# zhaoyuhsin/Edge-Guided-Near-Eye-Image-Analysis-for-Head-Mounted-Displays

Measured on AMD Instinct MI355X. Metric: eye-frames/sec (320x240): inference edge+seg (value), +fit, exact fp32, and train fwd+bwd at 1 MI355X, higher is better.
Workload: dtype f32 tensors; inference products split into f16 hi/lo pairs (3 f16 MFMAs per product, 22-bit significand), f32 accumulate (`exact_fp32`: every product on the f32 MFMA); `train`: bf16 storage, f32 accumulate, f32 master weights (and an f32-storage leg)

## Files before the change

edge-guided-near-eye-image-analysis-for-head-mounted-displays_amd/csrc/conv1x1_f16.hip:

```cpp
#include "common.h"
#include "kernel_util.h"
#include "split_f16.h"

namespace {

__device__ __forceinline__ void split8(const u32x4 a, const u32x4 b, float s, h8& hi, h8& lo) {
  const f32x4 va = __builtin_bit_cast(f32x4, a), vb = __builtin_bit_cast(f32x4, b);
  const float x[8] = {va[0], va[1], va[2], va[3], vb[0], vb[1], vb[2], vb[3]};
#pragma unroll
  for (int q = 0; q < 4; ++q) {
    h2 h, l;
    egne::split2(x[2 * q], x[2 * q + 1], s, h, l);
    hi[2 * q] = h[0]; hi[2 * q + 1] = h[1];
    lo[2 * q] = l[0]; lo[2 * q + 1] = l[1];
  }
}

template <int TN, bool UP = false>
__global__ __launch_bounds__(256) void conv1x1_f16x3_kernel(const egne_conv_desc p, const _Float16* __restrict__ fhi,
                                                            const _Float16* __restrict__ flo, float a_scale, float out_scale,
                                                            int G, long long M, int nblocks) {
  extern __shared__ __attribute__((aligned(16))) _Float16 wl[];
  const int tid = threadIdx.x, lane = tid & 63, wave = tid >> 6;
  const int li = lane & 31, kq = lane >> 5;
  const int NT = p.CoutP >> 5, nt0 = blockIdx.y * TN;
  for (int it = tid; it < G * TN * 2 * 64; it += 256) {
    const int l = it & 63, hl = (it >> 6) & 1;
    const int tn = (it >> 7) % TN, g = (it >> 7) / TN;
    const _Float16* src = (hl ? flo : fhi) + (((long long)g * NT + nt0 + tn) * 64 + l) * 8;
    *(u32x4*)&wl[(long long)it * 8] = *(const u32x4*)src;
  }
  __syncthreads();
  constexpr int UPC = 18, UPP = 32 * TN + 8;
  [[maybe_unused]] float* const patch = (float*)(wl + (long long)G * TN * 2 * 64 * 8) + wave * (UPC * UPP);

  const float slope = p.act == EGNE_ACT_RELU ? 0.f : (p.act == EGNE_ACT_LEAKY ? 0.01f : 1.f);
  f32x4 bias[TN][4];
#pragma unroll
  for (int tn = 0; tn < TN; ++tn)
#pragma unroll
    for (int j = 0; j < 4; ++j) {
      const int n = (nt0 + tn) * 32 + 8 * j + 4 * kq;
      bias[tn][j] = (p.bias && n < p.Cout_store) ? *(const f32x4*)(p.bias + n) : (f32x4)(0.f);
    }

  for (int blk = blockIdx.x * 4 + wave; blk < nblocks; blk += gridDim.x * 4) {
    const long long m0 = (long long)blk * 32;
    const long long rows = M - m0 < 32 ? M - m0 : 32;
    f32x16 acc[TN];
#pragma unroll
    for (int tn = 0; tn < TN; ++tn) acc[tn] = (f32x16)(0.f);
    int g = 0;
    for (int s = 0; s < p.nseg; ++s) {
      const egne_seg sg = p.seg[s];
      const __amdgpu_buffer_rsrc_t r = make_rsrc(sg.ptr + m0 * sg.pix_stride, (unsigned)(rows * sg.pix_stride * 4));
      const int voff = (li * (int)sg.pix_stride + sg.ch_off + 4 * kq) * 4;
      const int n16 = (sg.Cp + 15) >> 4;
      const bool tail8 = (sg.Cp & 15) != 0;
      for (int g0 = 0; g0 < n16; g0 += 4) {
        u32x4 xa[4], xb[4];
#pragma unroll
        for (int u = 0; u < 4; ++u) {
          const int gg = g0 + u;
          const int oa = gg < n16 ? voff : (int)OOB;
          const int ob = (gg < n16 && !(tail8 && gg == n16 - 1)) ? voff : (int)OOB;
          xa[u] = __builtin_amdgcn_raw_buffer_load_b128(r, oa, gg * 64, 0);
          xb[u] = __builtin_amdgcn_raw_buffer_load_b128(r, ob + 32, gg * 64, 0);
        }
#pragma unroll
        for (int u = 0; u < 4; ++u) {
          if (g0 + u < n16) {
            h8 ah, al;
            split8(xa[u], xb[u], a_scale, ah, al);
            const _Float16* wp = wl + ((long long)(g + g0 + u) * TN * 2 * 64 + lane) * 8;
#pragma unroll
            for (int tn = 0; tn < TN; ++tn) {
              const h8 wh = *(const h8*)(wp + (tn * 2 + 0) * 512), wo = *(const h8*)(wp + (tn * 2 + 1) * 512);
              acc[tn] = __builtin_amdgcn_mfma_f32_32x32x16_f16(wh, al, acc[tn], 0, 0, 0);
              acc[tn] = __builtin_amdgcn_mfma_f32_32x32x16_f16(wo, ah, acc[tn], 0, 0, 0);
              acc[tn] = __builtin_amdgcn_mfma_f32_32x32x16_f16(wh, ah, acc[tn], 0, 0, 0);
            }
          }
        }
      }
      g += n16;
    }
    const __amdgpu_buffer_rsrc_t ro = make_rsrc(p.out + m0 * p.out_pix_stride, (unsigned)(rows * p.out_pix_stride * 4));
    bool bad = false;
    [[maybe_unused]] int o00 = 0, o01 = 0, o10 = 0, o11 = 0;
    [[maybe_unused]] float w00 = 0.f, w01 = 0.f, w10 = 0.f, w11 = 0.f;
    [[maybe_unused]] __amdgpu_buffer_rsrc_t rres = ro;
    [[maybe_unused]] bool pix_ok = false, staged = false;
    if constexpr (UP) {
      const int ph = p.Ho, pw = p.Wo, hw = p.H * p.W;
      const long long m = m0 + li;
      pix_ok = m < M;
      const int b = pix_ok ? (int)(m / hw) : 0;
      const int r = pix_ok ? (int)(m - (long long)b * hw) : 0;
      const int y = r / p.W, x = r - y * p.W;
      float sy = 0.5f * (y + 0.5f) - 0.5f, sx = 0.5f * (x + 0.5f) - 0.5f;
      sy = sy < 0.f ? 0.f : sy; sx = sx < 0.f ? 0.f : sx;
      const int y0 = (int)sy, x0 = (int)sx, y1 = y0 + (y0 < ph - 1 ? 1 : 0), x1 = x0 + (x0 < pw - 1 ? 1 : 0);
      const float ly = sy - y0, lx = sx - x0;
      w00 = (1.f - ly) * (1.f - lx); w01 = (1.f - ly) * lx; w10 = ly * (1.f - lx); w11 = ly * lx;
      const int rs = (int)p.res_pix_stride, base = b * ph * pw;
      rres = make_rsrc(p.residual, (unsigned)((long long)p.B * ph * pw * rs * 4));
      const int r0 = (int)(m0 % hw), xb0 = r0 % p.W;
      staged = rows == 32 && xb0 + 32 <= p.W;
      if (staged) {
        const int bb = (int)(m0 / hw), yb = r0 / p.W;
        float syb = 0.5f * (yb + 0.5f) - 0.5f; syb = syb < 0.f ? 0.f : syb;
        const int yb0 = (int)syb, yb1 = yb0 + (yb0 < ph - 1 ? 1 : 0);
        const float lyb = syb - yb0;
        float sxb = 0.5f * (xb0 + 0.5f) - 0.5f; sxb = sxb < 0.f ? 0.f : sxb;
        const int cb = (int)sxb;
        constexpr int VPP = 8 * TN;
        for (int it = lane; it < UPC * VPP; it += 64) {
          const int cc = it / VPP, c4 = it - cc * VPP;
          const int gx = cb + cc < pw ? cb + cc : pw - 1;
          const int n = nt0 * 32 + c4 * 4;
          const int o0 = n < p.Cout_store ? (((bb * ph + yb0) * pw + gx) * rs + p.res_ch_off + n) * 4 : (int)OOB;
          const int o1 = n < p.Cout_store ? (((bb * ph + yb1) * pw + gx) * rs + p.res_ch_off + n) * 4 : (int)OOB;
          const f32x4 ra = __builtin_bit_cast(f32x4, __builtin_amdgcn_raw_buffer_load_b128(rres, o0, 0, 0));
          const f32x4 rb = __builtin_bit_cast(f32x4, __builtin_amdgcn_raw_buffer_load_b128(rres, o1, 0, 0));
          *(f32x4*)&patch[cc * UPP + c4 * 4] = (1.f - lyb) * ra + lyb * rb;
        }
        asm volatile("s_waitcnt vmcnt(0) lgkmcnt(0)" ::: "memory");
        o00 = ((x0 - cb) * UPP) * 4; o01 = ((x1 - cb) * UPP) * 4;
        w00 = 1.f - lx; w01 = lx;
      } else {
        o00 = ((base + y0 * pw + x0) * rs + p.res_ch_off) * 4; o01 = ((base + y0 * pw + x1) * rs + p.res_ch_off) * 4;
        o10 = ((base + y1 * pw + x0) * rs + p.res_ch_off) * 4; o11 = ((base + y1 * pw + x1) * rs + p.res_ch_off) * 4;
      }
    }
#pragma unroll
    for (int tn = 0; tn < TN; ++tn)
#pragma unroll
      for (int j = 0; j < 4; ++j) {
        const int n = (nt0 + tn) * 32 + 8 * j + 4 * kq;
        f32x4 v;
#pragma unroll
        for (int e = 0; e < 4; ++e) {
          const float t = acc[tn][4 * j + e] * out_scale + bias[tn][j][e];
          v[e] = fmaxf(t, t * slope);
        }
        if (tn == 0 && j == 0) bad |= egne_nonfinite(v[0]);
        if constexpr (UP) {
          if (staged) {
            const char* pb = (const char*)patch + (tn * 32 + 8 * j + 4 * kq) * 4;
            v += w00 * *(const f32x4*)(pb + o00) + w01 * *(const f32x4*)(pb + o01);
          } else {
          const bool on = pix_ok && n < p.Cout_store;
          const f32x4 a = __builtin_bit_cast(f32x4, __builtin_amdgcn_raw_buffer_load_b128(rres, on ? o00 + n * 4 : (int)OOB, 0, 0));
          const f32x4 b_ = __builtin_bit_cast(f32x4, __builtin_amdgcn_raw_buffer_load_b128(rres, on ? o01 + n * 4 : (int)OOB, 0, 0));
          const f32x4 c = __builtin_bit_cast(f32x4, __builtin_amdgcn_raw_buffer_load_b128(rres, on ? o10 + n * 4 : (int)OOB, 0, 0));
          const f32x4 d_ = __builtin_bit_cast(f32x4, __builtin_amdgcn_raw_buffer_load_b128(rres, on ? o11 + n * 4 : (int)OOB, 0, 0));
          v += w00 * a + w01 * b_ + w10 * c + w11 * d_;
          }
        }
        const int off = n < p.Cout_store ? (li * (int)p.out_pix_stride + p.out_ch_off + n) * 4 : (int)OOB;
        __builtin_amdgcn_raw_buffer_store_b128(__builtin_bit_cast(u32x4, v), ro, off, 0, 0);
      }
    egne_ovf_commit(bad, p.ovf_flag);
  }
}


template <int TN, bool STATS = false>
__global__ __launch_bounds__(256) void conv1x1_pool_f16x3_kernel(const egne_conv_desc p, const _Float16* __restrict__ fhi,
                                                                 const _Float16* __restrict__ flo, float a_scale, float out_scale,
                                                                 int G, long long M, int nblocks) {
  extern __shared__ __attribute__((aligned(16))) _Float16 wl[];
  const int tid = threadIdx.x, lane = tid & 63, wave = tid >> 6;
  const int li = lane & 31, kq = lane >> 5;
  const int NT = p.CoutP >> 5, nt0 = blockIdx.y * TN;
  for (int it = tid; it < G * TN * 2 * 64; it += 256) {
    const int l = it & 63, hl = (it >> 6) & 1;
    const int tn = (it >> 7) % TN, g = (it >> 7) / TN;
    const _Float16* src = (hl ? flo : fhi) + (((long long)g * NT + nt0 + tn) * 64 + l) * 8;
    *(u32x4*)&wl[(long long)it * 8] = *(const u32x4*)src;
  }
  __syncthreads();

  const float slope = p.act == EGNE_ACT_RELU ? 0.f : (p.act == EGNE_ACT_LEAKY ? 0.01f : 1.f);
  [[maybe_unused]] f32x4 bias[STATS ? 1 : TN][4];
  if constexpr (!STATS) {
#pragma unroll
  for (int tn = 0; tn < TN; ++tn)
#pragma unroll
    for (int j = 0; j < 4; ++j) {
      const int n = (nt0 + tn) * 32 + 8 * j + 4 * kq;
      bias[tn][j] = (p.bias && n < p.Cout_store) ? *(const f32x4*)(p.bias + n) : (f32x4)(0.f);
    }
  }
  const int H = p.H, W = p.W, Hp = p.Ho, Wp = p.Wo, hwp = Hp * Wp;
  const float s4 = 0.25f * a_scale;

  constexpr bool stats = STATS;
  const int bpf = (hwp + 31) >> 5, cb = stats ? (bpf + p.stats_nchunk - 1) / p.stats_nchunk : 1;
  constexpr int PP = 36;
  [[maybe_unused]] float* const patch = (float*)(wl + (long long)G * TN * 2 * 64 * 8) + wave * (32 * PP);
  [[maybe_unused]] const int rd = (lane >> 5) * PP + (lane & 31);

  for (int unit = blockIdx.x * 4 + wave; unit < nblocks; unit += gridDim.x * 4) {
   long long mfirst = (long long)unit * 32, mend = M;
   if (stats) {
     const int fb = unit / p.stats_nchunk, ck = unit - fb * p.stats_nchunk;
     mfirst = (long long)fb * hwp + (long long)ck * cb * 32;
     mend = (long long)(fb + 1) * hwp;
   }
   if (mend > mfirst + (long long)cb * 32) mend = mfirst + (long long)cb * 32;
   [[maybe_unused]] double ssum[TN], qsum[TN];
#pragma unroll
   for (int tn = 0; tn < TN; ++tn) ssum[tn] = qsum[tn] = 0.;
   for (long long m0 = mfirst; m0 < mend; m0 += 32) {
    const long long rows = mend - m0 < 32 ? mend - m0 : 32;
    const int b0 = (int)(m0 / hwp);
    const long long m = m0 + li;
    const bool valid = li < rows;
    const int b = valid ? (int)(m / hwp) : b0;
    const int r = (int)(m - (long long)b * hwp);
    const int yp = valid ? r / Wp : 0, xp = valid ? r - yp * Wp : 0;
    const int pin = ((b - b0) * H + 2 * yp) * W + 2 * xp;
    f32x16 acc[TN];
#pragma unroll
    for (int tn = 0; tn < TN; ++tn) acc[tn] = (f32x16)(0.f);
    int g = 0;
    for (int s = 0; s < p.nseg; ++s) {
      const egne_seg sg = p.seg[s];
      const long long frame = (long long)H * W * sg.pix_stride;
      const long long left = ((long long)p.B - b0) * frame * 4;
      const __amdgpu_buffer_rsrc_t rs = make_rsrc(sg.ptr + (long long)b0 * frame, (unsigned)(left < 2 * frame * 4 ? left : 2 * frame * 4));
      const int ps4 = (int)sg.pix_stride * 4;
      const int voff = valid ? (pin * (int)sg.pix_stride + sg.ch_off + 4 * kq) * 4 : (int)OOB;
      const float slope_in = sg.act_in == EGNE_ACT_RELU ? 0.f : (sg.act_in == EGNE_ACT_LEAKY ? 0.01f : 1.f);
      const float* tsc = sg.scale + (long long)b * sg.Cp + 4 * kq;
      const float* tsh = sg.shift + (long long)b * sg.Cp + 4 * kq;
      const int n16 = (sg.Cp + 15) >> 4;
      const bool tail8 = (sg.Cp & 15) != 0;
      for (int gg = 0; gg < n16; ++gg) {
        const bool has_b = !(tail8 && gg == n16 - 1);
        const int ob = has_b ? voff + 32 : (int)OOB;
        u32x4 xa[4], xb[4];
#pragma unroll
        for (int t = 0; t < 4; ++t) {
          const int d = ((t >> 1) * W + (t & 1)) * ps4;
          xa[t] = __builtin_amdgcn_raw_buffer_load_b128(rs, voff == (int)OOB ? (int)OOB : voff + d, gg * 64, 0);
          xb[t] = __builtin_amdgcn_raw_buffer_load_b128(rs, ob == (int)OOB ? (int)OOB : ob + d, gg * 64, 0);
        }
        const f32x4 sca = *(const f32x4*)(tsc + gg * 16), sha = *(const f32x4*)(tsh + gg * 16);
        const f32x4 scb = has_b ? *(const f32x4*)(tsc + gg * 16 + 8) : (f32x4)(0.f), shb = has_b ? *(const f32x4*)(tsh + gg * 16 + 8) : (f32x4)(0.f);
        f32x4 sa = (f32x4)(0.f), sb = (f32x4)(0.f);
#pragma unroll
        for (int t = 0; t < 4; ++t) {
          f32x4 va = __builtin_bit_cast(f32x4, xa[t]) * sca + sha, vb = __builtin_bit_cast(f32x4, xb[t]) * scb + shb;
#pragma unroll
          for (int e = 0; e < 4; ++e) { sa[e] += fmaxf(va[e], va[e] * slope_in); sb[e] += fmaxf(vb[e], vb[e] * slope_in); }
        }
        if (!valid) { sa = (f32x4)(0.f); sb = (f32x4)(0.f); }
        h8 ah, al;
        split8(__builtin_bit_cast(u32x4, sa), __builtin_bit_cast(u32x4, sb), s4, ah, al);
        const _Float16* wp = wl + ((long long)(g + gg) * TN * 2 * 64 + lane) * 8;
#pragma unroll
        for (int tn = 0; tn < TN; ++tn) {
          const h8 wh = *(const h8*)(wp + (tn * 2 + 0) * 512), wo = *(const h8*)(wp + (tn * 2 + 1) * 512);
          acc[tn] = __builtin_amdgcn_mfma_f32_32x32x16_f16(wh, al, acc[tn], 0, 0, 0);
          acc[tn] = __builtin_amdgcn_mfma_f32_32x32x16_f16(wo, ah, acc[tn], 0, 0, 0);
          acc[tn] = __builtin_amdgcn_mfma_f32_32x32x16_f16(wh, ah, acc[tn], 0, 0, 0);
        }
      }
      g += n16;
    }
    const __amdgpu_buffer_rsrc_t ro = make_rsrc(p.out + m0 * p.out_pix_stride, (unsigned)(rows * p.out_pix_stride * 4));
    bool bad = false;
#pragma unroll
    for (int tn = 0; tn < TN; ++tn)
#pragma unroll
      for (int j = 0; j < 4; ++j) {
        const int n = (nt0 + tn) * 32 + 8 * j + 4 * kq;
        f32x4 v, bv;
        if constexpr (STATS) bv = (p.bias && n < p.Cout_store) ? *(const f32x4*)(p.bias + n) : (f32x4)(0.f);
        else bv = bias[tn][j];
#pragma unroll
        for (int e = 0; e < 4; ++e) {
          const float t = acc[tn][4 * j + e] * out_scale + bv[e];
          v[e] = fmaxf(t, t * slope);
        }
        if (tn == 0 && j == 0) bad |= egne_nonfinite(v[0]);
        const int off = n < p.Cout_store ? (li * (int)p.out_pix_stride + p.out_ch_off + n) * 4 : (int)OOB;
        __builtin_amdgcn_raw_buffer_store_b128(__builtin_bit_cast(u32x4, v), ro, off, 0, 0);
        if constexpr (stats) {
          *(f32x4*)&patch[li * PP + 8 * j + 4 * kq] = valid ? v : (f32x4)(0.f);
          if (j == 3) {
            asm volatile("s_waitcnt lgkmcnt(0)" ::: "memory");
            double s_ = ssum[tn], q_ = qsum[tn];
#pragma unroll
            for (int i = 0; i < 16; ++i) {
              const double x = (double)patch[i * 2 * PP + rd];
              s_ += x; q_ += x * x;
            }
            ssum[tn] = s_; qsum[tn] = q_;
          }
        }
      }
    egne_ovf_commit(bad, p.ovf_flag);
   }
   if constexpr (stats) {
#pragma unroll
     for (int tn = 0; tn < TN; ++tn) {
       const double s_ = ssum[tn] + __shfl_xor(ssum[tn], 32), q_ = qsum[tn] + __shfl_xor(qsum[tn], 32);
       const int n = (nt0 + tn) * 32 + lane;
       if (lane < 32 && n < p.Cout_store)
         ((double2*)p.stats_ws)[(long long)unit * p.Cout_store + n] = make_double2(s_, q_);
     }
   }
  }
}

__global__ void pack_w1x1_f16_k(const float* __restrict__ w, int Cout, int Cin, const int* __restrict__ kmap, int G, int CoutP,
                                float wscale, _Float16* __restrict__ hi, _Float16* __restrict__ lo) {
  const long long total = (long long)G * CoutP * 16;
  const int NT = CoutP >> 5;
  for (long long i = (long long)blockIdx.x * blockDim.x + threadIdx.x; i < total; i += (long long)gridDim.x * blockDim.x) {
    const int j = (int)(i & 7), nn = (int)((i >> 3) & 31), h = (int)((i >> 8) & 1);
    long long q = i >> 9;
    const int nt = (int)(q % NT);
    const int g = (int)(q / NT);
    const int n = nt * 32 + nn, ci = kmap[g * 16 + h * 8 + j];
    const float v = (n < Cout && ci >= 0) ? w[(long long)n * Cin + ci] * wscale : 0.f;
    const _Float16 hh = (_Float16)v;
    hi[i] = hh;
    lo[i] = (_Float16)(v - (float)hh);
  }
}

}

extern "C" int egne_pack_conv1x1_weight_f16(const float* w_oihw, int Cout, int Cin, const int32_t* kmap, int G, int CoutP,
                                            float wscale, void* fhi, void* flo, void* stream) {
  EGNE_REQUIRE(w_oihw && kmap && fhi && flo && Cout > 0 && Cin > 0 && G > 0 && CoutP >= Cout && CoutP % 32 == 0 && wscale > 0.f,
               "pack_conv1x1_f16: bad sizes Cout %d Cin %d G %d CoutP %d", Cout, Cin, G, CoutP);
  long long total = (long long)G * CoutP * 16, g = (total + 255) / 256;
  if (g > 4096) g = 4096;
  hipLaunchKernelGGL(pack_w1x1_f16_k, dim3((unsigned)g), dim3(256), 0, (hipStream_t)stream, w_oihw, Cout, Cin, kmap, G, CoutP, wscale,
                     (_Float16*)fhi, (_Float16*)flo);
  return egne::check_launch("egne_pack_conv1x1_weight_f16");
}

extern "C" int egne_conv1x1_f16x3_fwd(const egne_conv_desc* dp, const void* fhi, const void* flo, float a_scale, float w_scale,
                                      void* stream) {
  EGNE_REQUIRE(dp && fhi && flo, "conv1x1_f16: null pointer");
  const egne_conv_desc& d = *dp;
  EGNE_REQUIRE(egne::fp32_storage(d), "conv1x1_f16: split-pair / f16 storage (presplit, out_split) is not known here");
  const bool up = d.residual && d.Ho * 2 == d.H && d.Wo * 2 == d.W;
  EGNE_REQUIRE(d.kh == 1 && d.kw == 1 && d.stride == 1 && d.pad_h == 0 && d.pad_w == 0 && d.ngroups == 1 && (up || (d.Ho == d.H && d.Wo == d.W)) &&
               d.nseg >= 1 && d.nseg <= EGNE_MAXSEG && (up || !d.residual) && !d.post_scale, "conv1x1_f16: unsupported descriptor");
  EGNE_REQUIRE(!up || (d.act == EGNE_ACT_NONE && ((uintptr_t)d.residual & 15) == 0 && d.res_pix_stride % 4 == 0 && d.res_ch_off % 4 == 0 &&
                       d.res_ch_off + d.Cout_store <= d.res_pix_stride && (long long)d.B * d.Ho * d.Wo * d.res_pix_stride * 4 < (1ll << 31) &&
                       (long long)d.B * d.H * d.W < (1ll << 31)),
               "conv1x1_f16: up-sampled addend (no activation, 16-byte aligned channel vectors, < 2 GB)");
  EGNE_REQUIRE(d.CoutP % 32 == 0 && (d.CoutP == 32 || d.CoutP % 64 == 0) && d.Cout_store <= d.CoutP && d.Cout_store % 4 == 0 && d.out &&
               ((uintptr_t)d.out & 15) == 0 && d.out_pix_stride % 4 == 0 && d.out_ch_off % 4 == 0 &&
               d.out_ch_off + d.Cout_store <= d.out_pix_stride, "conv1x1_f16: output");
  EGNE_REQUIRE(!d.bias || ((uintptr_t)d.bias & 15) == 0, "conv1x1_f16: bias alignment");
  int G = 0;
  for (int s = 0; s < d.nseg; ++s) {
    const egne_seg& g = d.seg[s];
    EGNE_REQUIRE(g.ptr && !g.scale && !g.shift && g.act_in == EGNE_ACT_NONE && g.Cp % 8 == 0 && g.ch_off % 4 == 0 &&
                 g.pix_stride % 4 == 0 && ((uintptr_t)g.ptr & 15) == 0 && g.ch_off + g.Cp <= g.pix_stride && g.pix_stride * 128 < (1ll << 31),
                 "conv1x1_f16: slice %d", s);
    G += (g.Cp + 15) / 16;
  }
  EGNE_REQUIRE(d.out_pix_stride * 128 < (1ll << 31) && ((uintptr_t)fhi & 15) == 0 && ((uintptr_t)flo & 15) == 0 && a_scale > 0.f && w_scale > 0.f,
               "conv1x1_f16: strides / weights / scales");
  const long long M = (long long)d.B * d.H * d.W;
  const long long nb = (M + 31) / 32;
  EGNE_REQUIRE(nb < (1ll << 31), "conv1x1_f16: too many pixels");
  const int TN = d.CoutP == 32 ? 1 : 2;
  const size_t lds = (size_t)G * TN * 2 * 64 * 8 * sizeof(_Float16);
  EGNE_REQUIRE(lds <= 80 * 1024, "conv1x1_f16: K = %d groups of 16 does not fit the LDS weight image", G);
  if (!egne::raise_lds_all(80 * 1024, conv1x1_f16x3_kernel<1>, conv1x1_f16x3_kernel<2>))
    return egne::fail(EGNE_ERR_LAUNCH, "conv1x1_f16: cannot raise the dynamic LDS limit");
  const int ny = d.CoutP / (32 * TN);
  long long gx = (nb + 3) / 4;
  const long long cap = 256 * 8;
  if (gx > cap) gx = cap;
  const float os = 1.0f / (a_scale * w_scale);
  hipStream_t st = (hipStream_t)stream;
  if (up) {
    const size_t lds_up = lds + (size_t)4 * 18 * (32 * TN + 8) * sizeof(float);
    EGNE_REQUIRE(lds_up <= 80 * 1024, "conv1x1_f16: K = %d groups of 16 leaves no room for the addend patches", G);
    if (!egne::raise_lds_all(80 * 1024, conv1x1_f16x3_kernel<1, true>, conv1x1_f16x3_kernel<2, true>))
      return egne::fail(EGNE_ERR_LAUNCH, "conv1x1_f16: cannot raise the dynamic LDS limit");
    if (TN == 1)
      hipLaunchKernelGGL((conv1x1_f16x3_kernel<1, true>), dim3((unsigned)gx, ny), dim3(256), lds_up, st, d, (const _Float16*)fhi, (const _Float16*)flo,
                         a_scale, os, G, M, (int)nb);
    else
      hipLaunchKernelGGL((conv1x1_f16x3_kernel<2, true>), dim3((unsigned)gx, ny), dim3(256), lds_up, st, d, (const _Float16*)fhi, (const _Float16*)flo,
                         a_scale, os, G, M, (int)nb);
  } else if (TN == 1)
    hipLaunchKernelGGL((conv1x1_f16x3_kernel<1>), dim3((unsigned)gx, ny), dim3(256), lds, st, d, (const _Float16*)fhi, (const _Float16*)flo,
                       a_scale, os, G, M, (int)nb);
  else
    hipLaunchKernelGGL((conv1x1_f16x3_kernel<2>), dim3((unsigned)gx, ny), dim3(256), lds, st, d, (const _Float16*)fhi, (const _Float16*)flo,
                       a_scale, os, G, M, (int)nb);
  return egne::check_launch("egne_conv1x1_f16x3_fwd");
}

extern "C" int egne_conv1x1_pool2_f16x3_fwd(const egne_conv_desc* dp, const void* fhi, const void* flo, float a_scale, float w_scale,
                                            void* stream) {
  EGNE_REQUIRE(dp && fhi && flo, "conv1x1_pool2_f16: null pointer");
  const egne_conv_desc& d = *dp;
  EGNE_REQUIRE(egne::fp32_storage(d), "conv1x1_f16: split-pair / f16 storage (presplit, out_split) is not known here");
  EGNE_REQUIRE(d.kh == 1 && d.kw == 1 && d.stride == 1 && d.pad_h == 0 && d.pad_w == 0 && d.ngroups == 1 && d.Ho == d.H / 2 && d.Wo == d.W / 2 &&
               d.Ho > 0 && d.Wo > 0 && d.nseg >= 1 && d.nseg <= EGNE_MAXSEG && !d.residual && !d.post_scale, "conv1x1_pool2_f16: unsupported descriptor");
  EGNE_REQUIRE(d.CoutP % 32 == 0 && d.CoutP <= 96 && d.Cout_store <= d.CoutP && d.Cout_store % 4 == 0 && d.out &&
               ((uintptr_t)d.out & 15) == 0 && d.out_pix_stride % 4 == 0 && d.out_ch_off % 4 == 0 &&
               d.out_ch_off + d.Cout_store <= d.out_pix_stride && (!d.bias || ((uintptr_t)d.bias & 15) == 0), "conv1x1_pool2_f16: output");
  int G = 0;
  for (int s = 0; s < d.nseg; ++s) {
    const egne_seg& g = d.seg[s];
    EGNE_REQUIRE(g.ptr && g.scale && g.shift && ((uintptr_t)g.scale & 15) == 0 && ((uintptr_t)g.shift & 15) == 0 && g.Cp % 8 == 0 &&
                 g.ch_off % 4 == 0 && g.pix_stride % 4 == 0 && ((uintptr_t)g.ptr & 15) == 0 && g.ch_off + g.Cp <= g.pix_stride &&
                 (long long)d.H * d.W * g.pix_stride * 8 < (1ll << 31), "conv1x1_pool2_f16: slice %d", s);
    G += (g.Cp + 15) / 16;
  }
  EGNE_REQUIRE(d.out_pix_stride * 128 < (1ll << 31) && ((uintptr_t)fhi & 15) == 0 && ((uintptr_t)flo & 15) == 0 && a_scale > 0.f && w_scale > 0.f,
               "conv1x1_pool2_f16: strides / weights / scales");
  const long long M = (long long)d.B * d.Ho * d.Wo;
  const long long nb = (M + 31) / 32;
  EGNE_REQUIRE(nb < (1ll << 31), "conv1x1_pool2_f16: too many pixels");
  const int TN = d.CoutP / 32;
  const int bpf = (d.Ho * d.Wo + 31) / 32;
  EGNE_REQUIRE(!d.stats_ws || (((uintptr_t)d.stats_ws & 15) == 0 && d.stats_nchunk >= 1 && d.stats_nchunk <= bpf &&
                               (long long)(d.stats_nchunk - 1) * ((bpf + d.stats_nchunk - 1) / d.stats_nchunk) < bpf &&
                               (long long)d.B * d.stats_nchunk < (1ll << 31)),
               "conv1x1_pool2_f16: stats_ws needs 1 <= stats_nchunk <= %d blocks per frame, no empty chunk", bpf);
  const size_t lds = (size_t)G * TN * 2 * 64 * 8 * sizeof(_Float16) + (d.stats_ws ? (size_t)4 * 32 * 36 * sizeof(float) : 0);
  EGNE_REQUIRE(lds <= 80 * 1024, "conv1x1_pool2_f16: K = %d groups of 16 does not fit the LDS weight image", G);
  if (!egne::raise_lds_all(80 * 1024, conv1x1_pool_f16x3_kernel<1>, conv1x1_pool_f16x3_kernel<2>, conv1x1_pool_f16x3_kernel<3>,
                           conv1x1_pool_f16x3_kernel<1, true>, conv1x1_pool_f16x3_kernel<2, true>, conv1x1_pool_f16x3_kernel<3, true>))
    return egne::fail(EGNE_ERR_LAUNCH, "conv1x1_pool2_f16: cannot raise the dynamic LDS limit");
  const int ny = 1;
  const long long nu = d.stats_ws ? (long long)d.B * d.stats_nchunk : nb;
  long long gx = (nu + 3) / 4;
  const long long cap = 256 * 8;
  if (gx > cap) gx = cap;
  const float os = 1.0f / (a_scale * w_scale);
  hipStream_t st = (hipStream_t)stream;
  const dim3 grid((unsigned)gx, (unsigned)ny);
  const _Float16* h = (const _Float16*)fhi;
  const _Float16* l = (const _Float16*)flo;
  if (d.stats_ws) {
    if (TN == 1) hipLaunchKernelGGL((conv1x1_pool_f16x3_kernel<1, true>), grid, dim3(256), lds, st, d, h, l, a_scale, os, G, M, (int)nu);
    else if (TN == 2) hipLaunchKernelGGL((conv1x1_pool_f16x3_kernel<2, true>), grid, dim3(256), lds, st, d, h, l, a_scale, os, G, M, (int)nu);
    else hipLaunchKernelGGL((conv1x1_pool_f16x3_kernel<3, true>), grid, dim3(256), lds, st, d, h, l, a_scale, os, G, M, (int)nu);
  } else if (TN == 1) hipLaunchKernelGGL((conv1x1_pool_f16x3_kernel<1>), grid, dim3(256), lds, st, d, h, l, a_scale, os, G, M, (int)nu);
  else if (TN == 2) hipLaunchKernelGGL((conv1x1_pool_f16x3_kernel<2>), grid, dim3(256), lds, st, d, h, l, a_scale, os, G, M, (int)nu);
  else hipLaunchKernelGGL((conv1x1_pool_f16x3_kernel<3>), grid, dim3(256), lds, st, d, h, l, a_scale, os, G, M, (int)nu);
  return egne::check_launch("egne_conv1x1_pool2_f16x3_fwd");
}
```

Measured before the change: 2172.

## Stream 1x1-conv activations through a per-wave LDS DMA ring buffer

Adds a DMA variant of the f16x3 1x1 conv kernel. Each wave keeps a ring of up to four 8 KB slots in LDS and fills them with buffer_load_lds, issuing activation tiles for future K-chunks and pixel blocks ahead of use, with swizzled addresses to avoid bank conflicts. For the fused upsample-add path, the bilinear addend patch is also loaded by DMA into swizzled LDS instead of through registers. The intent is to hide global load latency behind the MFMAs. In exchange it uses far more LDS (up to 160 KB), which lowers blocks per CU and caps the grid. It is on by default and can be turned off with the EGNE_S1X1_DMA environment variable.

```diff
diff --git a/edge-guided-near-eye-image-analysis-for-head-mounted-displays_amd/csrc/conv1x1_f16.hip b/edge-guided-near-eye-image-analysis-for-head-mounted-displays_amd/csrc/conv1x1_f16.hip
--- a/edge-guided-near-eye-image-analysis-for-head-mounted-displays_amd/csrc/conv1x1_f16.hip
+++ b/edge-guided-near-eye-image-analysis-for-head-mounted-displays_amd/csrc/conv1x1_f16.hip
@@ -3,6 +3,19 @@
 #include "split_f16.h"
 
 namespace {
+
+constexpr int S1X1_UNIT = 8192, S1X1_MAXRING = 4;
+__host__ __device__ constexpr int s1x1_np(int TN) { return (2 * 18 * 8 * TN + 63) / 64; }
+__host__ __device__ constexpr size_t s1x1_ring_off(int G, int TN, bool up) {
+  return (size_t)G * TN * 2048 + (up ? (size_t)4 * s1x1_np(TN) * 1024 : 0);
+}
+template <int X = 0>
+__device__ __forceinline__ void s1x1_wait_units(int n) {
+  if (n >= 3) asm volatile("s_waitcnt vmcnt(%0)" ::"n"(24 + X) : "memory");
+  else if (n == 2) asm volatile("s_waitcnt vmcnt(%0)" ::"n"(16 + X) : "memory");
+  else if (n == 1) asm volatile("s_waitcnt vmcnt(%0)" ::"n"(8 + X) : "memory");
+  else asm volatile("s_waitcnt vmcnt(%0)" ::"n"(X) : "memory");
+}
 
 __device__ __forceinline__ void split8(const u32x4 a, const u32x4 b, float s, h8& hi, h8& lo) {
   const f32x4 va = __builtin_bit_cast(f32x4, a), vb = __builtin_bit_cast(f32x4, b);
@@ -16,12 +29,13 @@
   }
 }
 
-template <int TN, bool UP = false>
+template <int TN, bool UP = false, bool DMA = false>
 __global__ __launch_bounds__(256) void conv1x1_f16x3_kernel(const egne_conv_desc p, const _Float16* __restrict__ fhi,
                                                             const _Float16* __restrict__ flo, float a_scale, float out_scale,
-                                                            int G, long long M, int nblocks) {
-  extern __shared__ __attribute__((aligned(16))) _Float16 wl[];
-  const int tid = threadIdx.x, lane = tid & 63, wave = tid >> 6;
+                                                            int G, long long M, int nblocks, int NR) {
+  extern __shared__ __attribute__((aligned(1024))) _Float16 wl[];
+  const int tid = threadIdx.x, lane = tid & 63;
+  const int wave = DMA ? __builtin_amdgcn_readfirstlane(tid >> 6) : tid >> 6;
   const int li = lane & 31, kq = lane >> 5;
   const int NT = p.CoutP >> 5, nt0 = blockIdx.y * TN;
   for (int it = tid; it < G * TN * 2 * 64; it += 256) {
@@ -44,21 +58,96 @@
       bias[tn][j] = (p.bias && n < p.Cout_store) ? *(const f32x4*)(p.bias + n) : (f32x4)(0.f);
     }
 
+  [[maybe_unused]] char* const ring = (char*)wl + s1x1_ring_off(G, TN, UP) + wave * NR * S1X1_UNIT;
+  [[maybe_unused]] const int lp = lane >> 4;
+  [[maybe_unused]] const int bstride = gridDim.x * 4;
+  [[maybe_unused]] int pb = blockIdx.x * 4 + wave, psg = 0, pg0 = 0, pslot = 0, cslot = 0, ahead = 0;
+  [[maybe_unused]] int since = 0;
+  [[maybe_unused]] auto issue = [&]() {
+    if (pb >= nblocks) return;
+    const egne_seg sg = p.seg[psg];
+    const long long m0 = (long long)pb * 32;
+    const int rows = M - m0 < 32 ? (int)(M - m0) : 32;
+    const int ps = (int)sg.pix_stride;
+    const __amdgpu_buffer_rsrc_t r = make_rsrc(sg.ptr + m0 * ps, (unsigned)(rows * ps * 4));
+    const int base = (lp * ps + sg.ch_off + pg0 * 16) * 4;
+    char* const dst = ring + pslot * S1X1_UNIT;
+#pragma unroll
+    for (int i = 0; i < 8; ++i) {
+      const int c = (lane & 15) ^ (4 * (i & 3) + lp);
+      const bool ok = pg0 * 16 + c * 4 < sg.Cp && 4 * i + lp < rows;
+      __builtin_amdgcn_raw_ptr_buffer_load_lds(r, (lds_ptr)(dst + i * 1024), 16, ok ? base + i * 16 * ps + c * 16 : (int)OOB, 0, 0, 0);
+    }
+    pg0 += 4;
+    if (pg0 * 16 >= sg.Cp) {
+      pg0 = 0;
+      if (++psg == p.nseg) { psg = 0; pb += bstride; }
+    }
+    ++ahead;
+    ++since;
+    if (++pslot == NR) pslot = 0;
+  };
+  constexpr int NP = s1x1_np(TN), VPP = 8 * TN;
+  [[maybe_unused]] char* const praw = (char*)wl + (long long)G * TN * 2048 + wave * (NP * 1024);
+  auto pkey = [](int cc) { return TN == 2 ? (cc & 15) : ((cc >> 1) & 7); };
+  [[maybe_unused]] int pexp = 0;
+  [[maybe_unused]] const int rda = li * 256 + ((kq ^ (li & 15)) << 4), rdb = li * 256 + (((2 | kq) ^ (li & 15)) << 4);
+  if constexpr (DMA)
+    for (int i = 0; i < NR; ++i) issue();
+
   for (int blk = blockIdx.x * 4 + wave; blk < nblocks; blk += gridDim.x * 4) {
     const long long m0 = (long long)blk * 32;
     const long long rows = M - m0 < 32 ? M - m0 : 32;
     f32x16 acc[TN];
 #pragma unroll
     for (int tn = 0; tn < TN; ++tn) acc[tn] = (f32x16)(0.f);
+    if constexpr (UP && DMA) {
+      const int ph = p.Ho, pw = p.Wo, hw = p.H * p.W;
+      const int r0 = (int)(m0 % hw), xb0 = r0 % p.W;
+      if (rows == 32 && xb0 + 32 <= p.W) {
+        const int bb = (int)(m0 / hw), yb = r0 / p.W;
+        float syb = 0.5f * (yb + 0.5f) - 0.5f; syb = syb < 0.f ? 0.f : syb;
+        const int yb0 = (int)syb, yb1 = yb0 + (yb0 < ph - 1 ? 1 : 0);
+        float sxb = 0.5f * (xb0 + 0.5f) - 0.5f; sxb = sxb < 0.f ? 0.f : sxb;
+        const int cb = (int)sxb, rs = (int)p.res_pix_stride;
+        const __amdgpu_buffer_rsrc_t rres = make_rsrc(p.residual, (unsigned)((long long)p.B * ph * pw * rs * 4));
+        asm volatile("s_waitcnt lgkmcnt(0)" ::: "memory");
+#pragma unroll
+        for (int k = 0; k < NP; ++k) {
+          const int it = k * 64 + lane, row = it >= UPC * VPP ? 1 : 0, rem = it - row * (UPC * VPP);
+          const int cc = rem / VPP, c4 = (rem - cc * VPP) ^ pkey(cc);
+          const int gx = cb + cc < pw ? cb + cc : pw - 1;
+          const int n = nt0 * 32 + c4 * 4;
+          const bool ok = it < 2 * UPC * VPP && n < p.Cout_store;
+          const int o = (((bb * ph + (row ? yb1 : yb0)) * pw + gx) * rs + p.res_ch_off + n) * 4;
+          __builtin_amdgcn_raw_ptr_buffer_load_lds(rres, (lds_ptr)(praw + k * 1024), 16, ok ? o : (int)OOB, 0, 0, 0);
+        }
+        pexp = ahead;
+        since = 0;
+      }
+    }
     int g = 0;
     for (int s = 0; s < p.nseg; ++s) {
       const egne_seg sg = p.seg[s];
-      const __amdgpu_buffer_rsrc_t r = make_rsrc(sg.ptr + m0 * sg.pix_stride, (unsigned)(rows * sg.pix_stride * 4));
-      const int voff = (li * (int)sg.pix_stride + sg.ch_off + 4 * kq) * 4;
+      [[maybe_unused]] const __amdgpu_buffer_rsrc_t r = make_rsrc(sg.ptr + m0 * sg.pix_stride, (unsigned)(rows * sg.pix_stride * 4));
+      [[maybe_unused]] const int voff = (li * (int)sg.pix_stride + sg.ch_off + 4 * kq) * 4;
       const int n16 = (sg.Cp + 15) >> 4;
-      const bool tail8 = (sg.Cp & 15) != 0;
+      [[maybe_unused]] const bool tail8 = (sg.Cp & 15) != 0;
       for (int g0 = 0; g0 < n16; g0 += 4) {
         u32x4 xa[4], xb[4];
+        if constexpr (DMA) {
+          if (UP && pexp > 0) {
+            s1x1_wait_units<UP ? NP : 0>(ahead - 1);
+            --pexp;
+          } else
+            s1x1_wait_units(ahead - 1);
+          const char* const src = ring + cslot * S1X1_UNIT;
+#pragma unroll
+          for (int u = 0; u < 4; ++u) {
+            xa[u] = *(const u32x4*)(src + (rda ^ (u * 64)));
+            xb[u] = *(const u32x4*)(src + (rdb ^ (u * 64)));
+          }
+        } else {
 #pragma unroll
         for (int u = 0; u < 4; ++u) {
           const int gg = g0 + u;
@@ -66,6 +155,7 @@
           const int ob = (gg < n16 && !(tail8 && gg == n16 - 1)) ? voff : (int)OOB;
           xa[u] = __builtin_amdgcn_raw_buffer_load_b128(r, oa, gg * 64, 0);
           xb[u] = __builtin_amdgcn_raw_buffer_load_b128(r, ob + 32, gg * 64, 0);
+        }
         }
 #pragma unroll
         for (int u = 0; u < 4; ++u) {
@@ -82,6 +172,12 @@
             }
           }
         }
+        if constexpr (DMA) {
+          asm volatile("s_waitcnt lgkmcnt(0)" ::: "memory");
+          --ahead;
+          if (++cslot == NR) cslot = 0;
+          issue();
+        }
       }
       g += n16;
     }
@@ -91,6 +187,8 @@
     [[maybe_unused]] float w00 = 0.f, w01 = 0.f, w10 = 0.f, w11 = 0.f;
     [[maybe_unused]] __amdgpu_buffer_rsrc_t rres = ro;
     [[maybe_unused]] bool pix_ok = false, staged = false;
+    [[maybe_unused]] int k00 = 0, k01 = 0;
+    [[maybe_unused]] float lyb_ = 0.f;
     if constexpr (UP) {
       const int ph = p.Ho, pw = p.Wo, hw = p.H * p.W;
       const long long m = m0 + li;
@@ -114,7 +212,13 @@
         const float lyb = syb - yb0;
         float sxb = 0.5f * (xb0 + 0.5f) - 0.5f; sxb = sxb < 0.f ? 0.f : sxb;
         const int cb = (int)sxb;
-        constexpr int VPP = 8 * TN;
+        if constexpr (DMA) {
+          s1x1_wait_units(since);
+          lyb_ = lyb;
+          o00 = (x0 - cb) * (VPP * 16); o01 = (x1 - cb) * (VPP * 16);
+          k00 = pkey(x0 - cb) << 4; k01 = pkey(x1 - cb) << 4;
+          w00 = 1.f - lx; w01 = lx;
+        } else {
         for (int it = lane; it < UPC * VPP; it += 64) {
           const int cc = it / VPP, c4 = it - cc * VPP;
           const int gx = cb + cc < pw ? cb + cc : pw - 1;
@@ -128,6 +232,7 @@
         asm volatile("s_waitcnt vmcnt(0) lgkmcnt(0)" ::: "memory");
         o00 = ((x0 - cb) * UPP) * 4; o01 = ((x1 - cb) * UPP) * 4;
         w00 = 1.f - lx; w01 = lx;
+        }
       } else {
         o00 = ((base + y0 * pw + x0) * rs + p.res_ch_off) * 4; o01 = ((base + y0 * pw + x1) * rs + p.res_ch_off) * 4;
         o10 = ((base + y1 * pw + x0) * rs + p.res_ch_off) * 4; o11 = ((base + y1 * pw + x1) * rs + p.res_ch_off) * 4;
@@ -146,7 +251,16 @@
         }
         if (tn == 0 && j == 0) bad |= egne_nonfinite(v[0]);
         if constexpr (UP) {
-          if (staged) {
+          if (staged && DMA) {
+            const int c4 = (tn * 8 + 2 * j + kq) << 4;
+            const char* q0 = praw + o00 + (c4 ^ k00);
+            const char* q1 = praw + o01 + (c4 ^ k01);
+            const f32x4 ra0 = *(const f32x4*)q0, rb0 = *(const f32x4*)(q0 + UPC * VPP * 16);
+            const f32x4 ra1 = *(const f32x4*)q1, rb1 = *(const f32x4*)(q1 + UPC * VPP * 16);
+            const f32x4 p0 = (1.f - lyb_) * ra0 + lyb_ * rb0;
+            const f32x4 p1 = (1.f - lyb_) * ra1 + lyb_ * rb1;
+            v += w00 * p0 + w01 * p1;
+          } else if (staged) {
             const char* pb = (const char*)patch + (tn * 32 + 8 * j + 4 * kq) * 4;
             v += w00 * *(const f32x4*)(pb + o00) + w01 * *(const f32x4*)(pb + o01);
           } else {
@@ -383,27 +497,50 @@
     return egne::fail(EGNE_ERR_LAUNCH, "conv1x1_f16: cannot raise the dynamic LDS limit");
   const int ny = d.CoutP / (32 * TN);
   long long gx = (nb + 3) / 4;
+  const float os = 1.0f / (a_scale * w_scale);
+  hipStream_t st = (hipStream_t)stream;
+  const size_t lds_up = lds + (size_t)4 * 18 * (32 * TN + 8) * sizeof(float);
+  EGNE_REQUIRE(!up || lds_up <= 80 * 1024, "conv1x1_f16: K = %d groups of 16 leaves no room for the addend patches", G);
+  const char* e = getenv("EGNE_S1X1_DMA");
+  const int want = e ? atoi(e) : 1;
+  const size_t roff = s1x1_ring_off(G, TN, up), ring1 = (size_t)4 * S1X1_UNIT, lds_max = 160 * 1024;
+  int NR = 0;
+  if (want == 1) NR = S1X1_MAXRING;
+  else if (want >= 2) NR = want < S1X1_MAXRING ? want : S1X1_MAXRING;
+  while (NR >= 2 && roff + NR * ring1 > lds_max) --NR;
+  if (NR >= 2) {
+    const size_t lds_dma = roff + NR * ring1;
+    if (!egne::raise_lds_all(lds_max, conv1x1_f16x3_kernel<1, false, true>, conv1x1_f16x3_kernel<2, false, true>,
+                             conv1x1_f16x3_kernel<1, true, true>, conv1x1_f16x3_kernel<2, true, true>))
+      return egne::fail(EGNE_ERR_LAUNCH, "conv1x1_f16: cannot raise the dynamic LDS limit");
+    const long long cap = 256 * (lds_dma <= 80 * 1024 ? 2 : 1) / ny;
+    if (gx > cap) gx = cap > 0 ? cap : 1;
+    const dim3 grid((unsigned)gx, ny);
+    const _Float16* h = (const _Float16*)fhi;
+    const _Float16* l = (const _Float16*)flo;
+    if (up && TN == 1) hipLaunchKernelGGL((conv1x1_f16x3_kernel<1, true, true>), grid, dim3(256), lds_dma, st, d, h, l, a_scale, os, G, M, (int)nb, NR);
+    else if (up) hipLaunchKernelGGL((conv1x1_f16x3_kernel<2, true, true>), grid, dim3(256), lds_dma, st, d, h, l, a_scale, os, G, M, (int)nb, NR);
+    else if (TN == 1) hipLaunchKernelGGL((conv1x1_f16x3_kernel<1, false, true>), grid, dim3(256), lds_dma, st, d, h, l, a_scale, os, G, M, (int)nb, NR);
+    else hipLaunchKernelGGL((conv1x1_f16x3_kernel<2, false, true>), grid, dim3(256), lds_dma, st, d, h, l, a_scale, os, G, M, (int)nb, NR);
+    return egne::check_launch("egne_conv1x1_f16x3_fwd");
+  }
   const long long cap = 256 * 8;
   if (gx > cap) gx = cap;
-  const float os = 1.0f / (a_scale * w_scale);
-  hipStream_t st = (hipStream_t)stream;
   if (up) {
-    const size_t lds_up = lds + (size_t)4 * 18 * (32 * TN + 8) * sizeof(float);
-    EGNE_REQUIRE(lds_up <= 80 * 1024, "conv1x1_f16: K = %d groups of 16 leaves no room for the addend patches", G);
     if (!egne::raise_lds_all(80 * 1024, conv1x1_f16x3_kernel<1, true>, conv1x1_f16x3_kernel<2, true>))
       return egne::fail(EGNE_ERR_LAUNCH, "conv1x1_f16: cannot raise the dynamic LDS limit");
     if (TN == 1)
       hipLaunchKernelGGL((conv1x1_f16x3_kernel<1, true>), dim3((unsigned)gx, ny), dim3(256), lds_up, st, d, (const _Float16*)fhi, (const _Float16*)flo,
-                         a_scale, os, G, M, (int)nb);
+                         a_scale, os, G, M, (int)nb, 0);
     else
       hipLaunchKernelGGL((conv1x1_f16x3_kernel<2, true>), dim3((unsigned)gx, ny), dim3(256), lds_up, st, d, (const _Float16*)fhi, (const _Float16*)flo,
-                         a_scale, os, G, M, (int)nb);
+                         a_scale, os, G, M, (int)nb, 0);
   } else if (TN == 1)
     hipLaunchKernelGGL((conv1x1_f16x3_kernel<1>), dim3((unsigned)gx, ny), dim3(256), lds, st, d, (const _Float16*)fhi, (const _Float16*)flo,
-                       a_scale, os, G, M, (int)nb);
+                       a_scale, os, G, M, (int)nb, 0);
   else
     hipLaunchKernelGGL((conv1x1_f16x3_kernel<2>), dim3((unsigned)gx, ny), dim3(256), lds, st, d, (const _Float16*)fhi, (const _Float16*)flo,
-                       a_scale, os, G, M, (int)nb);
+                       a_scale, os, G, M, (int)nb, 0);
   return egne::check_launch("egne_conv1x1_f16x3_fwd");
 }
 
```

After: 2171. No clear change (-0.0%).
